# Shahriar1638/Hybrid-Language-Music-Clustering-VAE

Hardware: AMD Instinct MI355X
Metric: clips/sec mel+VAE train step, 128-mel x 128-frame, bs=256, 1/2/4/8 MI355X (higher is better)
Workload: dtype bf16; 1 GPU; Convolutional_VAE audio-only (BASELINE config[1]): PCM[256,65024] -> HIP mel-dB 128x128 -> z-score -> VAE fwd+bwd+Adam; per_gpu_batch=256, global_batch=256, mel=128x128, params=13304961, parallelism=dp1, world_size=1, launch=single process, pcm_batches=5 distinct batches in rotation (333 MB), execution=eager launches

## Files before the change

hybrid-language-music-clustering-vae_amd/_lib.py:

```python
from __future__ import annotations

import ctypes as C
import os

import torch

_HERE = os.path.dirname(os.path.abspath(__file__))
LIB_PATH = os.environ.get("HLMC_LIB") or os.path.join(_HERE, "libhlmc.so")

c_int, c_i64, c_f32, c_f64, c_vp, c_char_p = C.c_int, C.c_int64, C.c_float, C.c_double, C.c_void_p, C.c_char_p
P_vp = C.POINTER(c_vp)
P_i64 = C.POINTER(c_i64)

HLMC_F32, HLMC_BF16 = 0, 1
NET_HYBRID, NET_CVAE, NET_SIMPLE = 0, 1, 2

_SIGS = {
    "hlmc_version": (c_int, []),
    "hlmc_last_error": (c_char_p, []),
    "hlmc_device_status": (c_int, [c_int]),
    "hlmc_test_bn_fused": (c_int, [c_i64, c_int]),
    "hlmc_mel_plan_create": (c_int, [c_int, c_int, c_int, c_int, c_f64, c_f64, P_vp]),
    "hlmc_mel_plan_destroy": (c_int, [c_vp]),
    "hlmc_mel_filterbank": (c_int, [c_vp, c_vp]),
# ... 42 lines not shown
    "hlmc_probe_arm": (c_int, [c_int, c_int]),
    "hlmc_probe_read": (c_int, [C.POINTER(c_int), C.POINTER(c_f64), C.POINTER(c_f64), C.POINTER(c_f64),
                                C.POINTER(c_f32), c_int]),
    "hlmc_loss_workspace": (c_i64, [c_i64, c_i64, c_i64]),
    "hlmc_loss_sums": (c_int, [c_vp, c_vp, c_vp, c_i64, c_vp, c_vp, c_i64, c_vp, c_vp, c_i64, c_vp, c_vp]),
    "hlmc_loss_backward": (c_int, [c_vp, c_vp, c_vp, c_i64, c_vp, c_vp, c_vp, c_i64, c_vp, c_vp, c_vp, c_i64,
                                   c_vp, c_vp, c_vp]),
    "hlmc_loss_sums_backward": (c_int, [c_vp, c_vp, c_vp, c_i64, c_vp, c_vp, c_vp, c_i64, c_vp, c_vp, c_vp, c_i64,
                                        c_vp, c_vp, c_vp, c_vp, c_vp]),
    "hlmc_adam_scratch_bytes": (c_i64, [c_int]),
    "hlmc_adam_step": (c_int, [c_vp, c_int, P_vp, P_vp, P_vp, P_vp, P_i64, c_f32, c_f32, c_f32, c_f32, c_f32,
                               c_int, c_vp]),
    "hlmc_km_center": (c_int, [c_vp, c_vp, c_i64, c_int, c_vp, c_vp, c_vp]),
    "hlmc_km_sqdist_rows": (c_int, [c_vp, c_vp, c_i64, c_int, P_i64, c_int, c_vp]),
    "hlmc_km_assign": (c_int, [c_vp, c_vp, c_i64, c_int, c_vp, c_int, c_vp, c_vp, c_vp]),
    "hlmc_km_sums": (c_int, [c_vp, c_vp, c_i64, c_int, c_vp, c_int, c_vp, c_vp]),
    "hlmc_km_sums_workspace": (c_i64, [c_i64, c_int]),
    "hlmc_km_sums_part": (c_int, [c_vp, c_vp, c_i64, c_int, c_vp, c_int, c_vp, c_vp, c_vp, c_i64]),
    "hlmc_km_rowdist": (c_int, [c_vp, c_vp, c_i64, c_int, c_vp, c_vp, c_vp]),
    "hlmc_km_inertia": (c_int, [c_vp, c_vp, c_i64, c_int, c_vp, c_vp, c_vp, c_vp]),
    "hlmc_op_bn_bwd_workspace": (c_i64, [c_int]),
    "hlmc_op_bn_bwd": (c_int, [c_vp, c_int, c_vp, c_vp, c_i64, c_int, c_vp, c_vp, c_vp, c_vp, c_vp, c_vp, c_vp, c_vp, c_vp,
                               c_i64]),
    "hlmc_km_assign_batch": (c_int, [c_vp, c_vp, c_i64, c_int, c_vp, c_int, c_int, C.c_uint64, c_vp, c_vp, c_vp]),
    "hlmc_km_sums_batch": (c_int, [c_vp, c_vp, c_i64, c_int, c_vp, c_int, c_int, C.c_uint64, c_vp, c_vp, c_vp, c_i64]),
    "hlmc_km_update_batch": (c_int, [c_vp, c_int, c_int, c_int, C.c_uint64, c_vp, c_vp, c_vp, c_vp, c_vp]),
    "hlmc_km_pp_search": (c_int, [c_vp, c_i64, c_int, c_int, c_vp, c_int, C.POINTER(C.c_int32), C.POINTER(c_f64), c_vp,
                                  c_vp]),
    "hlmc_km_pp_dist": (c_int, [c_vp, c_vp, c_i64, c_int, c_int, c_int, c_vp, c_vp, c_int, C.POINTER(C.c_int32), c_vp]),
    "hlmc_km_inertia_batch": (c_int, [c_vp, c_vp, c_i64, c_int, c_vp, c_int, c_vp, c_int, c_vp, c_vp]),
    "hlmc_silhouette_workspace": (c_i64, [c_i64, c_int]),
    "hlmc_silhouette": (c_int, [c_vp, c_vp, c_i64, c_int, c_vp, c_int, c_vp, c_vp, c_vp, c_i64]),
    "hlmc_cluster_scores_workspace": (c_i64, [c_int, c_int]),
    "hlmc_cluster_scores": (c_int, [c_vp, c_vp, c_i64, c_int, c_vp, c_int, c_vp, c_vp, c_i64]),
    "hlmc_dbscan_workspace": (c_i64, [c_i64, c_int]),
    "hlmc_dbscan_neighbors": (c_int, [c_vp, c_vp, c_i64, c_int, C.POINTER(c_f64), c_int, c_vp, c_vp, c_vp, c_i64]),
    "hlmc_dbscan_labels": (c_int, [c_vp, c_i64, c_int, c_int, c_int, c_vp, c_vp, c_i64, c_vp, c_vp, c_vp]),
    "hlmc_ward_workspace": (c_i64, [c_i64]),
    "hlmc_ward_pdist": (c_int, [c_vp, c_vp, c_i64, c_int, c_vp]),
    "hlmc_ward_chain": (c_int, [c_vp, c_i64, c_vp, c_vp, c_vp, c_vp, c_vp, c_vp, c_i64]),
    "hlmc_op_conv_s2": (c_int, [c_vp, c_int, c_vp, c_int, c_int, c_int, c_int, c_vp, c_vp, c_int, c_vp, c_vp, c_i64]),
    "hlmc_op_subpixel": (c_int, [c_vp, c_int, c_vp, c_int, c_int, c_int, c_int, c_vp, c_vp, c_int, c_vp, c_vp, c_i64]),
    "hlmc_op_wgrad_s2": (c_int, [c_vp, c_int, c_vp, c_int, c_int, c_int, c_int, c_vp, c_int, c_vp, c_vp, c_i64]),
    "hlmc_op_linear": (c_int, [c_vp, c_int, c_vp, c_int, c_int, c_int, c_vp, c_int, c_vp, c_int, c_vp, c_int, c_int,
                               c_int, c_int, c_vp, c_i64, c_vp]),
    "hlmc_op_linear_wgrad": (c_int, [c_vp, c_int, c_vp, c_int, c_vp, c_int, c_int, c_int, c_int, c_vp, c_vp, c_vp,
# ... 78 lines not shown
```

hybrid-language-music-clustering-vae_amd/csrc/capi.cpp:

```cpp
#include <algorithm>
#include <cmath>
#include <cstring>
#include <memory>
#include <vector>

#include "engine.hpp"
#include "features.hpp"

namespace hlmc {

static thread_local std::string g_err;
void set_error(const std::string& msg) { g_err = msg; }
const char* get_error() { return g_err.c_str(); }
static int device_status_ok() {
    const unsigned st = ops::dev_status_take(false);
    if (st == 0) return HLMC_OK;
    set_error("device status " + std::to_string(st) +
              (st & kDevBnCountTimeout ? ": a one-launch BatchNorm backward's grid-wide arrival count timed out (grid not "
                                         "co-resident); that launch's dgamma / dbeta / dy are NaN" : "") +
              " -- clear with hlmc_device_status(1)");
    return HLMC_EDEVICE;
}

namespace probe {
// ... 493 lines not shown
    if (C <= 0) return 0;
    return (int64_t)(((ops::bn_acc_bytes(C) + 255) & ~(size_t)255) + ((ops::bias_acc_bytes(C) + 255) & ~(size_t)255) +
                     2 * (size_t)C * sizeof(float));
}
int hlmc_op_bn_bwd(void* stream, int dtype, const void* da, const void* y, int64_t R, int C, const float* mean,
                   const float* invstd, const float* gamma, const float* beta, void* dy, float* dgamma, float* dbeta,
                   float* dbias, void* ws, int64_t ws_bytes) {
    HLMC_CHECK_ARG(da && y && mean && invstd && gamma && beta && dy && dgamma && dbeta && ws && R > 1 && C > 0,
                   "hlmc_op_bn_bwd: arguments");
    HLMC_CHECK_ARG(ws_bytes >= hlmc_op_bn_bwd_workspace(C), "hlmc_op_bn_bwd: workspace too small");
    HLMC_TRY(device_status_ok());
    hipStream_t s = S(stream);
    unsigned char* w = static_cast<unsigned char*>(ws);
    const size_t o1 = (ops::bn_acc_bytes(C) + 255) & ~(size_t)255, o2 = o1 + ((ops::bias_acc_bytes(C) + 255) & ~(size_t)255);
    HLMC_HIP(hipMemsetAsync(ws, 0, o2, s));
    XAcc mom{reinterpret_cast<unsigned long long*>(w), xacc_shards(C), 2 * C};
    XAcc bacc{reinterpret_cast<unsigned long long*>(w + o1), xacc_shards(C), C};
    float* sums = reinterpret_cast<float*>(w + o2);
    return DT_DISPATCH(dtype,
        ops::bn_act_bwd<float>(s, (const float*)da, C, (const float*)y, R, C, mean, invstd, gamma, beta, 0, nullptr,
                               1.f, (float*)dy, dgamma, dbeta, mom, nullptr, dbias ? bacc : XAcc{}, dbias, sums),
        ops::bn_act_bwd<bf16>(s, (const bf16*)da, C, (const bf16*)y, R, C, mean, invstd, gamma, beta, 0, nullptr, 1.f,
                              (bf16*)dy, dgamma, dbeta, mom, nullptr, dbias ? bacc : XAcc{}, dbias, sums));
}
static size_t halo_acc_off(int Ci) { return (XAcc::bytes(xacc_shards(Ci), 2 * Ci) + 255) & ~(size_t)255; }
int64_t hlmc_op_halo_workspace(int Ci, int Co) {
    return (int64_t)(halo_acc_off(Ci) + XAcc::bytes(xacc_shards(Co), 2 * Co));
}
int hlmc_op_halo_fwd(void* stream, int kind, const void* x, int B, int Hi, int Wi, int Ci, const void* wp,
                     const float* bias, int Co, void* y, double* out_sums, const float* gamma, const float* beta,
                     float* running_mean, float* running_var, int64_t* num_batches_tracked, float momentum, float eps,
                     float* mean_out, float* invstd_out, void* a_out, void* ws, int64_t ws_bytes) {
    HLMC_CHECK_ARG(kind == 0 || kind == 1, "hlmc_op_halo_fwd: kind 0 (conv_s2) or 1 (subpixel)");
    HLMC_CHECK_ARG(out_sums && ws && ws_bytes >= hlmc_op_halo_workspace(Ci, Co), "hlmc_op_halo_fwd: workspace / out_sums");
    const bool xin = gamma != nullptr;
    HLMC_CHECK_ARG(kind == 0 ? ops::conv_s2_takes_input_bn<bf16>(B, Hi, Wi, Ci, Co)
                             : ops::subpixel_takes_input_bn<bf16>(B, Hi, Wi, Ci, Co),
                   "hlmc_op_halo_fwd: not an LDS halo-tile shape");
    if (xin) HLMC_CHECK_ARG(beta && mean_out && invstd_out && a_out, "hlmc_op_halo_fwd: input BatchNorm arguments");
    hipStream_t s = S(stream);
    unsigned char* w = static_cast<unsigned char*>(ws);
    XAcc ain{reinterpret_cast<unsigned long long*>(w), xacc_shards(Ci), 2 * Ci};
    XAcc aout{reinterpret_cast<unsigned long long*>(w + halo_acc_off(Ci)), xacc_shards(Co), 2 * Co};
    HLMC_HIP(hipMemsetAsync(ws, 0, (size_t)hlmc_op_halo_workspace(Ci, Co), s));
    const int64_t R = (int64_t)B * Hi * Wi;
    ops::BnInput bi{};
// ... 20 lines not shown
```

hybrid-language-music-clustering-vae_amd/csrc/engine.cpp:

```cpp
#include "engine.hpp"

#include <algorithm>
#include <climits>
#include <cstdlib>
#include <functional>

namespace hlmc {
namespace {

constexpr float kBnEps = 1e-5f;
constexpr float kBnMomentum = 0.1f;
constexpr int ENC_CH[7] = {1, 32, 64, 128, 256, 512, 512};
constexpr int DEC_CH[7] = {512, 512, 256, 128, 64, 32, 1};

inline int pad8(int64_t n) { return (int)((n + 7) & ~int64_t(7)); }

struct WgradQueue {
    using Fn = std::function<int(hipStream_t, Ws)>;
    bool on = true;
    Ws ws_main{nullptr, 0};
    Ws ws_own{nullptr, 0};

    WgradQueue() = default;
    WgradQueue(const WgradQueue&) = delete;
// ... 442 lines not shown
        int C = 0;
        float* gb = nullptr;
    };
    int bn_bwd(hipStream_t s, const T* da, int lda, const T* y, int64_t R, int C, const BnBufs& bb, int g, int beta,
               int act, const uint8_t* mask, float mscale, T* dy, int bias, const ops::BnBwdFuse* fused = nullptr,
               PendingBias* to_wgrad = nullptr) {
        const bool hand_off = bias >= 0 && wq.on && to_wgrad;
        const XAcc bacc = bias >= 0 ? acc_bias(bb) : XAcc{};
        if (to_wgrad) *to_wgrad = hand_off ? PendingBias{bacc, C, G[bias]} : PendingBias{};
        return ops::bn_act_bwd<T>(s, da, lda, y, R, C, AF(bb.mean), AF(bb.inv), P[g], P[beta], act, mask, mscale, dy,
                                  G[g], G[beta], acc_mom(bb), fused, bacc,
                                  (bias >= 0 && !hand_off) ? G[bias] : nullptr, AF(bb.sums));
    }
    ops::BnBwdFuse fuse4{};

    struct Enc {
        int w[6], b[6], g[6], beta[6], bn[6];
        int H = 0, W = 0;
        int rows(int l) const { return H >> l; }
        int cols(int l) const { return W >> l; }
        size_t y[6], a[6], dy[6];
        const float* audio = nullptr;
        BnBufs bb[6];
    };
    Enc enc;
    void enc_register(const std::string& prefix) {
        for (int l = 0; l < 6; ++l) {
            const int ci = ENC_CH[l], co = ENC_CH[l + 1];
            enc.w[l] = add_param(prefix + "." + std::to_string(3 * l) + ".weight", {co, ci, 3, 3});
            enc.b[l] = add_param(prefix + "." + std::to_string(3 * l) + ".bias", {co});
            enc.g[l] = add_param(prefix + "." + std::to_string(3 * l + 1) + ".weight", {co});
            enc.beta[l] = add_param(prefix + "." + std::to_string(3 * l + 1) + ".bias", {co});
            enc.bn[l] = add_bn();
            if (l > 0) register_pack(enc.w[l], 9);
        }
    }
    void enc_plan(Arena& A, int64_t B) {
        for (int l = 0; l < 6; ++l) {
            const int ci = ENC_CH[l], co = ENC_CH[l + 1];
            const int h = enc.rows(l), w = enc.cols(l), ho = enc.rows(l + 1), wo = enc.cols(l + 1);
            if (l > 0) {
                need(ops::conv_s2_ws<T>((int)B, h, w, ci, co));
                need(ops::subpixel_ws<T>((int)B, ho, wo, co, ci));
                need(ops::wgrad_s2_ws<T>((int)B, ho, wo, co, ci));
            } else {
                need(ops::wgrad_c1_ws((int)B, ho, wo, co));
            }
            const size_t n = (size_t)B * ho * wo * co;
            enc.y[l] = A.take(n * sizeof(T));
            enc.a[l] = l < 5 ? A.take(n * sizeof(T)) : 0;
            enc.dy[l] = A.take(n * sizeof(T));
            enc.bb[l] = bn_plan(A, co);
        }
    }
    size_t enc_max_elems(int64_t B) const { return (size_t)B * enc.rows(1) * enc.cols(1) * 32; }
    ops::BnInput bn_input(const BnBufs& bb, int bn, int g, int beta, int64_t R, size_t a_off) {
        return ops::BnInput{{acc_fwd(bb), R, AF(bb.mean), AF(bb.inv), RM[bn], RV[bn], NBT[bn], kBnMomentum, kBnEps},
                            P[g], P[beta], ws + a_off};
    }
    int enc_fwd(hipStream_t s, bool train, const float* audio_in, int B, T* flat, int ldflat) {
        HLMC_CHECK_ARG(audio_in, "audio input required");
        const float* audio = audio_in;
        enc.audio = audio_in;
        bool fused_prev = false;
        ops::BnInput xin{};
        for (int l = 0; l < 6; ++l) {
            const int ci = ENC_CH[l], co = ENC_CH[l + 1];
            const int h = enc.rows(l), w = enc.cols(l), ho = enc.rows(l + 1), wo = enc.cols(l + 1);
            T* y = AT(enc.y[l]);
            ops::ColStats st{train ? acc_fwd(enc.bb[l]) : XAcc{}, false};
            if (l == 0)
                HLMC_TRY(ops::conv_c1_s2<T>(s, audio, B, h, w, P[enc.w[0]], P[enc.b[0]], co, y, &st));
            else
                HLMC_TRY(ops::conv_s2<T>(s, fused_prev ? AT(enc.y[l - 1]) : AT(enc.a[l - 1]), B, h, w, ci, P0(enc.w[l]),
                                         P[enc.b[l]], co, y, scratch, &st, fused_prev ? &xin : nullptr));
            const int64_t R = (int64_t)B * ho * wo;
            fused_prev = train && l + 1 < 6 && ops::conv_s2_takes_input_bn<T>(B, ho, wo, co, ENC_CH[l + 2]);
            if (fused_prev) {
                if (!st.done) HLMC_TRY(ops::bn_moments<T>(s, y, R, co, acc_fwd(enc.bb[l])));
                xin = bn_input(enc.bb[l], enc.bn[l], enc.g[l], enc.beta[l], R, enc.a[l]);
            } else if (l == 5) {
                const ops::FlatOut fo{ldflat, nullptr};
                HLMC_TRY(bn_fwd(s, train, y, R, co, enc.bn[l], enc.bb[l], enc.g[l], enc.beta[l], 0, nullptr, 1.f, flat, 0,
                                &st, &fo, ho * wo));
            } else
                HLMC_TRY(bn_fwd(s, train, y, R, co, enc.bn[l], enc.bb[l], enc.g[l], enc.beta[l], 0, nullptr, 1.f,
                                AT(enc.a[l]), co, &st));
        }
        return HLMC_OK;
    }
    int enc_bwd(hipStream_t s, int B, T* gA, int bucket_hi = -1) {
        const float* audio = enc.audio;
        HLMC_CHECK_ARG(audio, "backward: no forward input recorded");
        for (int l = 5; l >= 0; --l) {
            const int ci = ENC_CH[l], co = ENC_CH[l + 1];
            const int ho = enc.rows(l + 1), wo = enc.cols(l + 1);
            const int64_t R = (int64_t)B * ho * wo;
            T* dy = AT(enc.dy[l]);
            PendingBias pb;
            HLMC_TRY(bn_bwd(s, gA, co, AT(enc.y[l]), R, co, enc.bb[l], enc.g[l], enc.beta[l], 0, nullptr, 1.f, dy, enc.b[l],
                            nullptr, &pb));
            float* gw = G[enc.w[l]];
            if (l == 0) {
                if (pb.gb) HLMC_TRY(ops::colsum_finalize(s, pb.acc, pb.C, pb.gb));
                HLMC_TRY(ops::wgrad_c1<T>(s, dy, B, ho, wo, co, audio, gw, scratch));
            } else {
                const T* xin = AT(enc.a[l - 1]);
                HLMC_TRY(wq.queue(s, [=](hipStream_t q, Ws sc) {
                    return ops::wgrad_s2<T>(q, dy, B, ho, wo, co, xin, ci, gw, sc, pb.acc, pb.gb);
                }, side_batch()));
                if (l == 1) HLMC_TRY(wq.flush(s));
                HLMC_TRY(ops::subpixel<T>(s, dy, B, ho, wo, co, P1(enc.w[l]), nullptr, ci, gA, scratch));
            }
            if (l == 3 && bucket_hi >= 0) HLMC_TRY(mark(s, bucket_hi));
            if (l == 2) HLMC_TRY(prelate(s));
        }
        return HLMC_OK;
    }

    struct Dec {
// ... 704 lines not shown
```

hybrid-language-music-clustering-vae_amd/csrc/kernels.hip:

```cpp
#include "ops.hpp"

#include <algorithm>
#include <cmath>
#include <cstdlib>
#include <cstring>
#include <map>
#include <mutex>
#include <tuple>
#include <type_traits>
#include <vector>
#include <atomic>

namespace hlmc {
namespace {

constexpr int kThreads = 256;
constexpr int kC1FusedBlocks = 1024;
constexpr int kC1BwdBlocks = 768;

inline int grid_for(int64_t n, int per_block = kThreads, int cap = 8192) {
    return (int)std::max<int64_t>(1, std::min<int64_t>(cap, (n + per_block - 1) / per_block));
}

constexpr int kBnBlockTarget = 1024;
// ... 974 lines not shown
            for (int j = 0; j < 9; ++j) red[wave][lane][i * 9 + j] = acc[i][j];
    }
    __syncthreads();
    for (int o = tid; o < M * 9; o += 256) {
        const int co = o / 9, tap = o - co * 9, g = co >> 3, i = co & 7;
        const float v = (red[0][g][i * 9 + tap] + red[1][g][i * 9 + tap]) + (red[2][g][i * 9 + tap] + red[3][g][i * 9 + tap]);
        part[(int64_t)blockIdx.x * (M * 9) + o] = v;
    }
}

__global__ __launch_bounds__(256) void sum_partials_f32_kernel(const float* __restrict__ part, int nblk, int n,
                                                               float* out) {
    __shared__ double sh[256];
    const int i = blockIdx.x;
    double s = 0.0;
    for (int k = threadIdx.x; k < nblk; k += blockDim.x) s += part[(int64_t)k * n + i];
    sh[threadIdx.x] = s;
    __syncthreads();
    for (int w = blockDim.x / 2; w > 0; w >>= 1) {
        if ((int)threadIdx.x < w) sh[threadIdx.x] += sh[threadIdx.x + w];
        __syncthreads();
    }
    if (threadIdx.x == 0) out[i] = (float)sh[0];
}

template <typename TI, typename TO>
__global__ void cast_kernel(const TI* __restrict__ x, TO* __restrict__ y, int64_t n) {
    for (int64_t i = (int64_t)blockIdx.x * blockDim.x + threadIdx.x; i < n; i += (int64_t)gridDim.x * blockDim.x)
        y[i] = from_f32<TO>(to_f32<TI>(x[i]));
}
template <typename TI, typename TO>
__global__ void cast2d_kernel(const TI* __restrict__ x, int ldx, TO* __restrict__ y, int ldy, int rows, int cols) {
    int64_t n = (int64_t)rows * cols;
    for (int64_t i = (int64_t)blockIdx.x * blockDim.x + threadIdx.x; i < n; i += (int64_t)gridDim.x * blockDim.x) {
        int r = (int)(i / cols), c = (int)(i % cols);
        y[(int64_t)r * ldy + c] = from_f32<TO>(to_f32<TI>(x[(int64_t)r * ldx + c]));
    }
}
struct LatentOut {
    float* mu = nullptr;
    float* lv = nullptr;
    float* eps = nullptr;
};
template <typename T>
__global__ void reparam_fwd_kernel(const float* __restrict__ mu, const float* __restrict__ lv,
                                   const float* __restrict__ eps, int n_rows, int L, T* __restrict__ z, int ldz,
// ... 740 lines not shown
        const int64_t rows = (int64_t)B * Hl;
        HLMC_CHECK_ARG(rows < (int64_t)1 << 31, "wgrad_c1: too many rows");
        const int nb = wgrad_c1_row_blocks(rows);
        HLMC_CHECK_ARG(ws.bytes >= (size_t)nb * M * 9 * sizeof(float), "wgrad_c1 workspace");
        wgrad_c1_rows_kernel<T><<<nb, kThreads, 0, s>>>(L, (int)rows, Hl, Xh, ws.p);
        HLMC_LAUNCHED();
        sum_partials_f32_kernel<<<M * 9, 256, 0, s>>>(ws.p, nb, M * 9, dW);
        HLMC_LAUNCHED();
        return HLMC_OK;
    }
    int64_t K = (int64_t)B * Hl * Wl;
    int nblk = wgrad_c1_blocks(K);
    HLMC_CHECK_ARG(ws.bytes >= wgrad_c1_ws(B, Hl, Wl, M), "wgrad_c1 workspace");
    int rpb = (int)((K + nblk - 1) / nblk);
    HLMC_CHECK_ARG(K < (int64_t)1 << 31, "wgrad_c1: too many rows");
    wgrad_c1_kernel<T, 32><<<nblk, kThreads, 0, s>>>(L, B, Hl, Wl, Xh, rpb, ws.p, FastDiv((uint32_t)Wl),
                                                     FastDiv((uint32_t)Hl));
    HLMC_LAUNCHED();
    sum_partials_f32_kernel<<<M * 9, 256, 0, s>>>(ws.p, nblk, M * 9, dW);
    HLMC_LAUNCHED();
    return HLMC_OK;
}

template <typename T>
int cast_from_f32(hipStream_t s, const float* x, T* y, int64_t n) {
    cast_kernel<float, T><<<grid_for(n), kThreads, 0, s>>>(x, y, n);
    HLMC_LAUNCHED();
    return HLMC_OK;
}
template <typename T>
int cast_to_f32(hipStream_t s, const T* x, float* y, int64_t n) {
    cast_kernel<T, float><<<grid_for(n), kThreads, 0, s>>>(x, y, n);
    HLMC_LAUNCHED();
    return HLMC_OK;
}
template <typename T>
int copy2d(hipStream_t s, const T* x, int ldx, T* y, int ldy, int rows, int cols) {
    cast2d_kernel<T, T><<<grid_for((int64_t)rows * cols), kThreads, 0, s>>>(x, ldx, y, ldy, rows, cols);
    HLMC_LAUNCHED();
    return HLMC_OK;
}
template <typename T>
int cast2d_from_f32(hipStream_t s, const float* x, int ldx, T* y, int ldy, int rows, int cols) {
    cast2d_kernel<float, T><<<grid_for((int64_t)rows * cols), kThreads, 0, s>>>(x, ldx, y, ldy, rows, cols);
    HLMC_LAUNCHED();
    return HLMC_OK;
// ... 229 lines not shown
int pack(hipStream_t s, const AdamJob* jobs_dev, int njobs, int total_tiles) {
    if (njobs == 0 || total_tiles == 0) return HLMC_OK;
    pack_kernel<T><<<total_tiles, 256, 0, s>>>(jobs_dev, njobs);
    HLMC_LAUNCHED();
    return HLMC_OK;
}

#define INST(T)                                                                                                      \
    template int bn_stats<T>(hipStream_t, const T*, int64_t, int, float*, float*, float*, float*, int64_t*, float,     \
                             float, XAcc);                                                                            \
    template int bn_moments<T>(hipStream_t, const T*, int64_t, int, XAcc);                                             \
    template int bn_act<T>(hipStream_t, const T*, int64_t, int, const float*, const float*, const float*, const float*, \
                           int, const uint8_t*, float, T*, int, const FlatOut*, int);                                 \
    template int bn_act_train<T>(hipStream_t, const T*, int64_t, int, XAcc, bool, float*, float*, float*,            \
                                 float*, int64_t*, float, float, const float*, const float*, int, const uint8_t*, float, \
                                 T*, int, const FlatOut*, int);                                                      \
    template int bn_act_bwd<T>(hipStream_t, const T*, int, const T*, int64_t, int, const float*, const float*,          \
                               const float*, const float*, int, const uint8_t*, float, T*, float*, float*, XAcc,      \
                               const BnBwdFuse*, XAcc, float*, float*);                                              \
    template int conv_c1_s2<T>(hipStream_t, const float*, int, int, int, const float*, const float*, int, T*,        \
                               ColStats*, BnBwdFuse*);                                                               \
    template int convT_c1<T>(hipStream_t, const T*, int, int, int, int, const float*, const float*, float*);         \
    template int wgrad_c1<T>(hipStream_t, const T*, int, int, int, int, const float*, float*, Ws);                    \
    template int cast_from_f32<T>(hipStream_t, const float*, T*, int64_t);                                           \
    template int cast_to_f32<T>(hipStream_t, const T*, float*, int64_t);                                             \
    template int copy2d<T>(hipStream_t, const T*, int, T*, int, int, int);                                           \
    template int cast2d_from_f32<T>(hipStream_t, const float*, int, T*, int, int, int);                              \
    template int heads_reparam<T>(hipStream_t, const float*, int, int, int, const float*, const float*, float*,      \
                                  float*, float*, float*, const float*, uint64_t, uint64_t, float*, T*, int);        \
    template int reparam_bwd_reduce<T>(hipStream_t, const float*, int, int, int, const float*, const float*,         \
                                       const float*, const float*, T*, T*, int);                                     \
    template int colsum<T>(hipStream_t, const T*, int, int, int, float*, Ws);                                        \
    template int reparam_fwd<T>(hipStream_t, const float*, const float*, const float*, int, int, T*, int, float*,     \
                                float*, float*);                                                                     \
    template int reparam_rng<T>(hipStream_t, const float*, const float*, uint64_t, uint64_t, int, int, float*, T*, int, \
                                float*, float*);                                                                     \
    template int reparam_bwd<T>(hipStream_t, const T*, int, const float*, const float*, const float*, const float*,  \
                                int, int, T*, T*);                                                                  \
    template int pack<T>(hipStream_t, const AdamJob*, int, int);                                                     \
    template int adam_pack<T>(hipStream_t, const AdamJob*, int, int, AdamArgs, const float*, int);

INST(float)
INST(bf16)
#undef INST

}
// ... 2 lines not shown
```

hybrid-language-music-clustering-vae_amd/csrc/ops.hpp:

```cpp
#pragma once
#include "common.hpp"

namespace hlmc {

struct Ws {
    float* p;
    size_t bytes;
};

namespace ops {

struct ColStats {
    XAcc acc;
    bool done;
};
struct BnBwdFuse {
    const void* y;
    const float *mean, *invstd, *gamma, *beta;
    XAcc acc;
    bool done;
};
struct BnInput : BnTrainFwd {
    const float *gamma = nullptr, *beta = nullptr;
    void* a_out = nullptr;
// ... 35 lines not shown
size_t linear_ws(int M, int K, int N);
template <typename T>
int linear_partials(hipStream_t s, const T* x, int ldx, int M, int K, const T* w, int ldw, int N, Ws ws, int* S_out);
template <typename T>
size_t linear_partials_ws(int M, int K, int N);

template <typename T>
int linear_wgrad(hipStream_t s, const T* dy, int lddy, const T* x, int ldx, int Mb, int N, int K, float* dW, float* db,
                 Ws ws);
template <typename T>
size_t linear_wgrad_ws(int Mb, int N, int K);
template <typename T>
int linear_wgrad_pair(hipStream_t s, const T* dy, int lddy, const T* x, int ldx, int Mb, int N1, int K, float* dW1,
                      float* db1, float* dW2, float* db2, Ws ws);

template <typename T>
int conv_c1_s2(hipStream_t s, const float* x, int B, int Hi, int Wi, const float* w, const float* bias, int Co, T* y,
               ColStats* st = nullptr, BnBwdFuse* bf = nullptr);
template <typename T>
int convT_c1(hipStream_t s, const T* x, int B, int Hi, int Wi, int Ci, const float* w, const float* bias, float* y);
template <typename T>
int wgrad_c1(hipStream_t s, const T* L, int B, int Hl, int Wl, int M, const float* Xh, float* dW, Ws ws);
size_t wgrad_c1_ws(int B, int Hl, int Wl, int M);

size_t bn_acc_bytes(int C);
size_t bias_acc_bytes(int C);
template <typename T>
int bn_stats(hipStream_t s, const T* y, int64_t R, int C, float* mean, float* invstd, float* run_mean, float* run_var,
             int64_t* nbt, float momentum, float eps, XAcc acc);
template <typename T>
int bn_moments(hipStream_t s, const T* y, int64_t R, int C, XAcc acc);
int bn_eval_stats(hipStream_t s, const float* run_mean, const float* run_var, int C, float eps, float* mean, float* invstd);
template <typename T>
int bn_act_train(hipStream_t s, const T* y, int64_t R, int C, XAcc acc, bool have_stats, float* mean, float* invstd,
                 float* run_mean, float* run_var, int64_t* nbt, float momentum, float eps, const float* gamma,
                 const float* beta, int act, const uint8_t* mask, float mscale, T* a, int lda,
                 const FlatOut* fo = nullptr, int hw = 0);
template <typename T>
int bn_act(hipStream_t s, const T* y, int64_t R, int C, const float* mean, const float* invstd, const float* gamma,
           const float* beta, int act, const uint8_t* mask, float mscale, T* a, int lda, const FlatOut* fo = nullptr,
           int hw = 0);
template <typename T>
int bn_act_bwd(hipStream_t s, const T* da, int lda, const T* y, int64_t R, int C, const float* mean, const float* invstd,
               const float* gamma, const float* beta, int act, const uint8_t* mask, float mscale, T* dy, float* dgamma,
               float* dbeta, XAcc mom, const BnBwdFuse* fused, XAcc bias_acc, float* dbias, float* sums);
int colsum_finalize(hipStream_t s, XAcc acc, int C, float* out);
// ... 72 lines not shown
```

include/hlmc.h:

```cpp
#ifndef HLMC_H_
#define HLMC_H_

#include <stdint.h>

#ifdef __cplusplus
extern "C" {
#endif

enum hlmc_status {
    HLMC_OK = 0,
    HLMC_EINVAL = -1,
    HLMC_EHIP = -2,
    HLMC_EUNSUP = -3,
    HLMC_EDEVICE = -4,
};

enum hlmc_dtype { HLMC_F32 = 0, HLMC_BF16 = 1 };

int hlmc_version(void);
const char* hlmc_last_error(void);
int hlmc_device_status(int clear);
int hlmc_test_bn_fused(int64_t max_elems, int spin_max);

typedef struct hlmc_mel_plan hlmc_mel_plan;
// ... 133 lines not shown


int hlmc_op_conv_s2(void* stream, int dtype, const void* x, int B, int Hi, int Wi, int Ci, const void* wp,
                    const float* bias, int Co, void* y, void* ws, int64_t ws_bytes);
int hlmc_op_subpixel(void* stream, int dtype, const void* x, int B, int Hi, int Wi, int Ci, const void* wp,
                     const float* bias, int Co, void* y, void* ws, int64_t ws_bytes);
int hlmc_op_wgrad_s2(void* stream, int dtype, const void* L, int B, int Hl, int Wl, int M, const void* Xh, int C,
                     float* dW, void* ws, int64_t ws_bytes);
int hlmc_op_linear(void* stream, int dtype, const void* x, int ldx, int M, int K, const void* w, int ldw,
                   const float* bias, int N, void* y, int ldy, int act, int accumulate, int out_f32, void* ws,
                   int64_t ws_bytes, const void* relu_ref);
int hlmc_op_linear_wgrad(void* stream, int dtype, const void* dy, int lddy, const void* x, int ldx, int Mb, int N,
                         int K, float* dW, float* db, void* ws, int64_t ws_bytes);
int hlmc_op_conv_c1_s2(void* stream, int dtype, const float* x, int B, int Hi, int Wi, const float* w,
                       const float* bias, int Co, void* y);
int hlmc_op_convT_c1(void* stream, int dtype, const void* x, int B, int Hi, int Wi, int Ci, const float* w,
                     const float* bias, float* y);
int hlmc_op_wgrad_c1(void* stream, int dtype, const void* L, int B, int Hl, int Wl, int M, const float* Xh,
                     float* dW, void* ws, int64_t ws_bytes);
int64_t hlmc_op_bn_bwd_workspace(int C);
int hlmc_op_bn_bwd(void* stream, int dtype, const void* da, const void* y, int64_t R, int C, const float* mean,
                   const float* invstd, const float* gamma, const float* beta, void* dy, float* dgamma, float* dbeta,
                   float* dbias, void* ws, int64_t ws_bytes);
int64_t hlmc_op_halo_workspace(int Ci, int Co);
int hlmc_op_halo_fwd(void* stream, int kind, const void* x, int B, int Hi, int Wi, int Ci, const void* wp,
                     const float* bias, int Co, void* y, double* out_sums, const float* gamma, const float* beta,
                     float* running_mean, float* running_var, int64_t* num_batches_tracked, float momentum, float eps,
                     float* mean_out, float* invstd_out, void* a_out, void* ws, int64_t ws_bytes);

#ifdef __cplusplus
}
#endif
#endif
```

Baseline: 144,200 clips/s.

## Fuse first-layer BN backward with conv weight-gradient via tap Gram algebra

For the first encoder layer (single input channel, 64-wide maps, 32 outputs), one row kernel now runs the BatchNorm backward and accumulates the per-tap products dz·x alongside the BN moment sums. The dy tensor is never written, and the separate weight-gradient pass over it is gone. The BN correction terms are applied afterwards in a single-block finalize kernel. That kernel uses a 9x9 Gram matrix of the input taps, computed on a side queue, to reconstruct the needed cross terms algebraically. This saves one full-size write and read of the layer-0 gradient at the cost of extra accumulators and a double-precision finalize with different rounding.

```diff
diff --git a/hybrid-language-music-clustering-vae_amd/_lib.py b/hybrid-language-music-clustering-vae_amd/_lib.py
--- a/hybrid-language-music-clustering-vae_amd/_lib.py
+++ b/hybrid-language-music-clustering-vae_amd/_lib.py
@@ -88,6 +88,9 @@
     "hlmc_op_bn_bwd_workspace": (c_i64, [c_int]),
     "hlmc_op_bn_bwd": (c_int, [c_vp, c_int, c_vp, c_vp, c_i64, c_int, c_vp, c_vp, c_vp, c_vp, c_vp, c_vp, c_vp, c_vp, c_vp,
                                c_i64]),
+    "hlmc_op_bn_bwd_wgrad_c1_workspace": (c_i64, []),
+    "hlmc_op_bn_bwd_wgrad_c1": (c_int, [c_vp, c_int, c_vp, c_vp, c_int, c_int, c_int, c_vp, c_vp, c_vp, c_vp, c_vp, c_vp,
+                                        c_vp, c_vp, c_vp, c_vp, c_vp, c_vp, c_i64]),
     "hlmc_km_assign_batch": (c_int, [c_vp, c_vp, c_i64, c_int, c_vp, c_int, c_int, C.c_uint64, c_vp, c_vp, c_vp]),
     "hlmc_km_sums_batch": (c_int, [c_vp, c_vp, c_i64, c_int, c_vp, c_int, c_int, C.c_uint64, c_vp, c_vp, c_vp, c_i64]),
     "hlmc_km_update_batch": (c_int, [c_vp, c_int, c_int, c_int, C.c_uint64, c_vp, c_vp, c_vp, c_vp, c_vp]),
diff --git a/hybrid-language-music-clustering-vae_amd/csrc/capi.cpp b/hybrid-language-music-clustering-vae_amd/csrc/capi.cpp
--- a/hybrid-language-music-clustering-vae_amd/csrc/capi.cpp
+++ b/hybrid-language-music-clustering-vae_amd/csrc/capi.cpp
@@ -539,6 +539,34 @@
                                1.f, (float*)dy, dgamma, dbeta, mom, nullptr, dbias ? bacc : XAcc{}, dbias, sums),
         ops::bn_act_bwd<bf16>(s, (const bf16*)da, C, (const bf16*)y, R, C, mean, invstd, gamma, beta, 0, nullptr, 1.f,
                               (bf16*)dy, dgamma, dbeta, mom, nullptr, dbias ? bacc : XAcc{}, dbias, sums));
+}
+static size_t al256(size_t b) { return (b + 255) & ~(size_t)255; }
+int64_t hlmc_op_bn_bwd_wgrad_c1_workspace(void) {
+    return (int64_t)(al256(ops::bn_acc_bytes(32)) + al256(ops::c1_bwd_acc_bytes()) + al256(ops::c1_gram_acc_bytes()));
+}
+int hlmc_op_bn_bwd_wgrad_c1(void* stream, int dtype, const void* da, const void* y, int B, int Hl, int Wl,
+                            const float* mean, const float* invstd, const float* gamma, const float* beta,
+                            const float* audio, const float* w, const float* bias, float* dW, float* dbias,
+                            float* dgamma, float* dbeta, void* ws, int64_t ws_bytes) {
+    HLMC_CHECK_ARG(da && y && mean && invstd && gamma && beta && audio && w && dW && dgamma && dbeta && ws,
+                   "hlmc_op_bn_bwd_wgrad_c1: arguments");
+    HLMC_CHECK_ARG(ws_bytes >= hlmc_op_bn_bwd_wgrad_c1_workspace(), "hlmc_op_bn_bwd_wgrad_c1: workspace too small");
+    HLMC_CHECK_ARG(DT_DISPATCH(dtype, ops::bn_bwd_wgrad_c1_ok<float>(B, Hl, Wl, 32, 0),
+                               ops::bn_bwd_wgrad_c1_ok<bf16>(B, Hl, Wl, 32, 0)),
+                   "hlmc_op_bn_bwd_wgrad_c1: only 64-wide maps");
+    hipStream_t s = S(stream);
+    unsigned char* p = static_cast<unsigned char*>(ws);
+    const size_t o1 = al256(ops::bn_acc_bytes(32)), o2 = o1 + al256(ops::c1_bwd_acc_bytes());
+    HLMC_HIP(hipMemsetAsync(ws, 0, (size_t)hlmc_op_bn_bwd_wgrad_c1_workspace(), s));
+    const XAcc mom{reinterpret_cast<unsigned long long*>(p), xacc_shards(32), 64};
+    const XAcc a = ops::c1_bwd_acc(p + o1), gram = ops::c1_gram_acc(p + o2);
+    HLMC_TRY(ops::c1_tap_gram(s, audio, B, Hl, Wl, gram));
+    HLMC_TRY(DT_DISPATCH(dtype,
+        ops::bn_bwd_wgrad_c1<float>(s, (const float*)da, (const float*)y, B, Hl, Wl, 32, mean, invstd, gamma, beta, 0,
+                                    audio, mom, a),
+        ops::bn_bwd_wgrad_c1<bf16>(s, (const bf16*)da, (const bf16*)y, B, Hl, Wl, 32, mean, invstd, gamma, beta, 0,
+                                   audio, mom, a)));
+    return ops::bn_bwd_c1_finalize(s, B, Hl, Wl, mom, a, gram, mean, invstd, gamma, w, bias, dW, dbias, dgamma, dbeta);
 }
 static size_t halo_acc_off(int Ci) { return (XAcc::bytes(xacc_shards(Ci), 2 * Ci) + 255) & ~(size_t)255; }
 int64_t hlmc_op_halo_workspace(int Ci, int Co) {
diff --git a/hybrid-language-music-clustering-vae_amd/csrc/engine.cpp b/hybrid-language-music-clustering-vae_amd/csrc/engine.cpp
--- a/hybrid-language-music-clustering-vae_amd/csrc/engine.cpp
+++ b/hybrid-language-music-clustering-vae_amd/csrc/engine.cpp
@@ -488,6 +488,8 @@
         size_t y[6], a[6], dy[6];
         const float* audio = nullptr;
         BnBufs bb[6];
+        bool one_pass0 = false;
+        size_t xa0 = 0, xgram0 = 0;
     };
     Enc enc;
     void enc_register(const std::string& prefix) {
@@ -515,8 +517,15 @@
             const size_t n = (size_t)B * ho * wo * co;
             enc.y[l] = A.take(n * sizeof(T));
             enc.a[l] = l < 5 ? A.take(n * sizeof(T)) : 0;
-            enc.dy[l] = A.take(n * sizeof(T));
+            if (l == 0) enc.one_pass0 = ops::bn_bwd_wgrad_c1_ok<T>((int)B, ho, wo, co, 0);
+            enc.dy[l] = l == 0 && enc.one_pass0 ? 0 : A.take(n * sizeof(T));
             enc.bb[l] = bn_plan(A, co);
+            if (l == 0 && enc.one_pass0) {
+                enc.xa0 = xb_total;
+                xb_total += al256(ops::c1_bwd_acc_bytes());
+                enc.xgram0 = xb_total;
+                xb_total += al256(ops::c1_gram_acc_bytes());
+            }
         }
     }
     size_t enc_max_elems(int64_t B) const { return (size_t)B * enc.rows(1) * enc.cols(1) * 32; }
@@ -558,10 +567,28 @@
     int enc_bwd(hipStream_t s, int B, T* gA, int bucket_hi = -1) {
         const float* audio = enc.audio;
         HLMC_CHECK_ARG(audio, "backward: no forward input recorded");
+        const XAcc gram0 = ops::c1_gram_acc(ws + xb_base + enc.xgram0);
+        if (enc.one_pass0) {
+            const int h1 = enc.rows(1), w1 = enc.cols(1);
+            HLMC_TRY(wq.run(s, [=](hipStream_t q, Ws) { return ops::c1_tap_gram(q, audio, B, h1, w1, gram0); }));
+        }
         for (int l = 5; l >= 0; --l) {
             const int ci = ENC_CH[l], co = ENC_CH[l + 1];
             const int ho = enc.rows(l + 1), wo = enc.cols(l + 1);
             const int64_t R = (int64_t)B * ho * wo;
+            if (l == 0 && enc.one_pass0) {
+                const BnBufs& bb = enc.bb[0];
+                const XAcc mom = acc_mom(bb), a0 = ops::c1_bwd_acc(ws + xb_base + enc.xa0);
+                const float *mean = AF(bb.mean), *inv = AF(bb.inv), *gam = P[enc.g[0]];
+                HLMC_TRY(ops::bn_bwd_wgrad_c1<T>(s, gA, AT(enc.y[0]), B, ho, wo, co, mean, inv, gam, P[enc.beta[0]], 0, audio,
+                                                 mom, a0));
+                const float *w0 = P[enc.w[0]], *b0 = P[enc.b[0]];
+                float *gw0 = G[enc.w[0]], *gb0 = G[enc.b[0]], *gg0 = G[enc.g[0]], *gbeta0 = G[enc.beta[0]];
+                HLMC_TRY(wq.run(s, [=](hipStream_t q, Ws) {
+                    return ops::bn_bwd_c1_finalize(q, B, ho, wo, mom, a0, gram0, mean, inv, gam, w0, b0, gw0, gb0, gg0, gbeta0);
+                }));
+                break;
+            }
             T* dy = AT(enc.dy[l]);
             PendingBias pb;
             HLMC_TRY(bn_bwd(s, gA, co, AT(enc.y[l]), R, co, enc.bb[l], enc.g[l], enc.beta[l], 0, nullptr, 1.f, dy, enc.b[l],
diff --git a/hybrid-language-music-clustering-vae_amd/csrc/kernels.hip b/hybrid-language-music-clustering-vae_amd/csrc/kernels.hip
--- a/hybrid-language-music-clustering-vae_amd/csrc/kernels.hip
+++ b/hybrid-language-music-clustering-vae_amd/csrc/kernels.hip
@@ -1020,6 +1020,222 @@
         __syncthreads();
     }
     if (threadIdx.x == 0) out[i] = (float)sh[0];
+}
+
+constexpr int kC1Taps = 9, kC1Co = 32;
+constexpr int kC1ACols = kC1Co * kC1Taps + kC1Co;
+constexpr int kC1GramCols = kC1Taps + kC1Taps * (kC1Taps + 1) / 2;
+constexpr int kC1Shards = 16;
+__host__ __device__ constexpr int c1_gram_col(int i, int j) {
+    const int a = i < j ? i : j, b = i < j ? j : i;
+    return kC1Taps + a * kC1Taps - a * (a - 1) / 2 + (b - a);
+}
+
+__device__ __forceinline__ void c1_load_taps(const float* __restrict__ Xh, int row, int Hl, int c, float (&xv)[3][3]) {
+    constexpr int WH = 128;
+    const int b = row / Hl, r = row - b * Hl;
+#pragma unroll
+    for (int kh = 0; kh < 3; ++kh) {
+        const int ih = 2 * r - 1 + kh;
+        const float* xr = Xh + ((int64_t)b * 2 * Hl + (ih < 0 ? 0 : ih)) * WH + 2 * c;
+        const float2 lo = *reinterpret_cast<const float2*>(xr - (c > 0 ? 2 : 0));
+        const float2 hi = *reinterpret_cast<const float2*>(xr);
+        const bool okr = ih >= 0;
+        xv[kh][0] = (okr && c > 0) ? lo.y : 0.f;
+        xv[kh][1] = okr ? hi.x : 0.f;
+        xv[kh][2] = okr ? hi.y : 0.f;
+    }
+}
+
+template <typename T>
+__global__ __launch_bounds__(256, 2) void bn_bwd_wgrad_c1_rows_kernel(
+    const T* __restrict__ da, const T* __restrict__ y, int rows, int Hl, const float* __restrict__ Xh,
+    const float* __restrict__ mean, const float* __restrict__ invstd, const float* __restrict__ gamma,
+    const float* __restrict__ beta, XAcc mom, XAcc aacc) {
+    constexpr int WL = 64, M = kC1Co, U = 4, NS = 8 * 9 + 3 * 8;
+    __shared__ double red[4][4][NS];
+    const int tid = threadIdx.x, c = tid >> 2, cg = tid & 3, lane = tid & 63, wave = tid >> 6;
+    float mu[8], is[8], ga[8], be[8];
+    BnChan::load(mean, 8 * cg, mu);
+    BnChan::load(invstd, 8 * cg, is);
+    BnChan::load(gamma, 8 * cg, ga);
+    BnChan::load(beta, 8 * cg, be);
+    float acc[8][9], fa[8], fb[8], fc[8];
+#pragma unroll
+    for (int i = 0; i < 8; ++i) {
+        fa[i] = fb[i] = fc[i] = 0.f;
+#pragma unroll
+        for (int j = 0; j < 9; ++j) acc[i][j] = 0.f;
+    }
+    const int stride = gridDim.x;
+    for (int r0 = blockIdx.x; r0 < rows; r0 += U * stride) {
+        float gv[U][8], yv[U][8], xv[U][3][3];
+#pragma unroll
+        for (int u = 0; u < U; ++u) {
+            const int row = r0 + u * stride < rows ? r0 + u * stride : 0;
+            const int64_t o = ((int64_t)row * WL + c) * M + 8 * cg;
+            if constexpr (sizeof(T) == 2) {
+                cvt16_f32<T>(load16_raw(da + o), gv[u]);
+                cvt16_f32<T>(load16_raw(y + o), yv[u]);
+            } else {
+                cvt16_f32<T>(load16_raw(da + o), gv[u]);
+                cvt16_f32<T>(load16_raw(da + o + 4), gv[u] + 4);
+                cvt16_f32<T>(load16_raw(y + o), yv[u]);
+                cvt16_f32<T>(load16_raw(y + o + 4), yv[u] + 4);
+            }
+            c1_load_taps(Xh, row, Hl, c, xv[u]);
+        }
+#pragma unroll
+        for (int u = 0; u < U; ++u) {
+            const bool valid = r0 + u * stride < rows;
+#pragma unroll
+            for (int i = 0; i < 8; ++i) {
+                float xh = (yv[u][i] - mu[i]) * is[i];
+                float z = xh * ga[i] + be[i];
+                float dz = gv[u][i] * act_grad_t<0>(z, 0);
+                dz = valid ? dz : 0.f;
+                fa[i] += dz;
+                fb[i] = fmaf(dz, xh, fb[i]);
+                fc[i] += valid ? xh : 0.f;
+#pragma unroll
+                for (int kh = 0; kh < 3; ++kh)
+#pragma unroll
+                    for (int kw = 0; kw < 3; ++kw) acc[i][kh * 3 + kw] = fmaf(dz, xv[u][kh][kw], acc[i][kh * 3 + kw]);
+            }
+        }
+    }
+#pragma unroll
+    for (int i = 0; i < 8; ++i)
+#pragma unroll
+        for (int j = 0; j < 9; ++j) {
+            double v = acc[i][j];
+#pragma unroll
+            for (int o = 4; o < 64; o <<= 1) v += __shfl_xor(v, o, 64);
+            if (lane < 4) red[wave][lane][i * 9 + j] = v;
+        }
+#pragma unroll
+    for (int i = 0; i < 8; ++i) {
+        double a = fa[i], b = fb[i], d = fc[i];
+#pragma unroll
+        for (int o = 4; o < 64; o <<= 1) {
+            a += __shfl_xor(a, o, 64);
+            b += __shfl_xor(b, o, 64);
+            d += __shfl_xor(d, o, 64);
+        }
+        if (lane < 4) {
+            red[wave][lane][72 + i] = a;
+            red[wave][lane][80 + i] = b;
+            red[wave][lane][88 + i] = d;
+        }
+    }
+    __syncthreads();
+    for (int o = tid; o < kC1ACols + 2 * M; o += 256) {
+        int co, slot;
+        if (o < M * 9) {
+            co = o / 9;
+            slot = (co & 7) * 9 + (o - co * 9);
+        } else {
+            const int k = (o - M * 9) / M;
+            co = (o - M * 9) - k * M;
+            slot = (k == 0 ? 88 : k == 1 ? 72 : 80) + (co & 7);
+        }
+        const int g = co >> 3;
+        const double v = (red[0][g][slot] + red[1][g][slot]) + (red[2][g][slot] + red[3][g][slot]);
+        if (o < kC1ACols)
+            xacc_add(aacc, o, v);
+        else
+            xacc_add(mom, o - kC1ACols, v);
+    }
+}
+
+__global__ __launch_bounds__(256) void c1_tap_gram_kernel(const float* __restrict__ Xh, int rows, int Hl, XAcc gacc) {
+    constexpr int NG = kC1GramCols;
+    __shared__ double red[4][NG];
+    const int tid = threadIdx.x, c = tid & 63, wave = tid >> 6;
+    float sx[9], pr[NG - 9];
+#pragma unroll
+    for (int i = 0; i < 9; ++i) sx[i] = 0.f;
+#pragma unroll
+    for (int i = 0; i < NG - 9; ++i) pr[i] = 0.f;
+    for (int row = blockIdx.x * 4 + wave; row < rows; row += gridDim.x * 4) {
+        float xv[3][3];
+        c1_load_taps(Xh, row, Hl, c, xv);
+        const float t[9] = {xv[0][0], xv[0][1], xv[0][2], xv[1][0], xv[1][1], xv[1][2], xv[2][0], xv[2][1], xv[2][2]};
+#pragma unroll
+        for (int i = 0; i < 9; ++i) {
+            sx[i] += t[i];
+#pragma unroll
+            for (int j = 0; j < 9; ++j)
+                if (j >= i) pr[c1_gram_col(i, j) - 9] = fmaf(t[i], t[j], pr[c1_gram_col(i, j) - 9]);
+        }
+    }
+#pragma unroll
+    for (int i = 0; i < 9; ++i) {
+        const double v = wave_sum((double)sx[i]);
+        if (c == 0) red[wave][i] = v;
+#pragma unroll
+        for (int j = 0; j < 9; ++j)
+            if (j >= i) {
+                const double p = wave_sum((double)pr[c1_gram_col(i, j) - 9]);
+                if (c == 0) red[wave][c1_gram_col(i, j)] = p;
+            }
+    }
+    __syncthreads();
+    if (tid < NG) xacc_add(gacc, tid, (red[0][tid] + red[1][tid]) + (red[2][tid] + red[3][tid]));
+}
+
+__device__ __forceinline__ double c1_xacc_column(const XAcc& acc, int c) {
+    unsigned long long w0[kC1Shards], w1[kC1Shards], w2[kC1Shards];
+#pragma unroll
+    for (int sh = 0; sh < kC1Shards; ++sh) {
+        const unsigned long long* q = acc.p + (size_t)sh * 3 * acc.ncols + c;
+        w0[sh] = q[0];
+        w1[sh] = q[acc.ncols];
+        w2[sh] = q[2 * acc.ncols];
+    }
+    long long a = 0, b = 0, d = 0;
+    unsigned long long bad = 0;
+#pragma unroll
+    for (int sh = 0; sh < kC1Shards; ++sh) {
+        a += (long long)w0[sh];
+        b += (long long)w1[sh];
+        bad |= w2[sh] & kXAccBad;
+        d += (long long)(w2[sh] & ~kXAccBad);
+    }
+    return bad ? __builtin_nan("") : xacc_value(a, b, d);
+}
+constexpr int kC1FinThreads = kC1ACols + 2 * kC1Co + 64;
+__global__ __launch_bounds__(kC1FinThreads) void bn_bwd_c1_finalize_kernel(XAcc mom, XAcc aacc, XAcc gacc, int64_t R,
+                                                                     const float* __restrict__ mean,
+                                                                     const float* __restrict__ invstd,
+                                                                     const float* __restrict__ gamma,
+                                                                     const float* __restrict__ w,
+                                                                     const float* __restrict__ bias, float* dW,
+                                                                     float* dbias, float* dgamma, float* dbeta) {
+    constexpr int M = kC1Co;
+    __shared__ double sa[kC1ACols], sm[2 * M], sg[kC1GramCols];
+    const int t = threadIdx.x;
+    if (t < kC1ACols)
+        sa[t] = c1_xacc_column(aacc, t);
+    else if (t < kC1ACols + 2 * M)
+        sm[t - kC1ACols] = c1_xacc_column(mom, t - kC1ACols);
+    else if (t < kC1ACols + 2 * M + kC1GramCols)
+        sg[t - kC1ACols - 2 * M] = c1_xacc_column(gacc, t - kC1ACols - 2 * M);
+    __syncthreads();
+    if (t >= kC1ACols) return;
+    const int c = t < M * 9 ? t / 9 : t - M * 9;
+    const double k = (double)gamma[c] * (double)invstd[c], mg = sm[c] / (double)R, mgx = sm[M + c] / (double)R;
+    if (t < M * 9) {
+        const int tap = t - c * 9;
+        double syx = (bias ? (double)bias[c] : 0.0) * sg[tap];
+        for (int j = 0; j < 9; ++j) syx += (double)w[c * 9 + j] * sg[c1_gram_col(j, tap)];
+        const double sxh = (double)invstd[c] * (syx - (double)mean[c] * sg[tap]);
+        dW[t] = (float)(k * (sa[t] - mg * sg[tap] - mgx * sxh));
+    } else {
+        dbeta[c] = (float)sm[c];
+        dgamma[c] = (float)sm[M + c];
+        if (dbias) dbias[c] = (float)(k * (sm[c] - (double)R * mg - mgx * sa[t]));
+    }
 }
 
 template <typename TI, typename TO>
@@ -1806,6 +2022,53 @@
     return HLMC_OK;
 }
 
+size_t c1_bwd_acc_bytes() { return XAcc::bytes(kC1Shards, kC1ACols); }
+size_t c1_gram_acc_bytes() { return XAcc::bytes(kC1Shards, kC1GramCols); }
+XAcc c1_bwd_acc(void* p) { return XAcc{static_cast<unsigned long long*>(p), kC1Shards, kC1ACols}; }
+XAcc c1_gram_acc(void* p) { return XAcc{static_cast<unsigned long long*>(p), kC1Shards, kC1GramCols}; }
+template <typename T>
+bool bn_bwd_wgrad_c1_ok(int B, int Hl, int Wl, int Co, int act) {
+    return B > 0 && Hl > 0 && Wl == 64 && Co == kC1Co && act == 0 && (int64_t)B * Hl < (int64_t)1 << 31;
+}
+int c1_tap_gram(hipStream_t s, const float* audio, int B, int Hl, int Wl, XAcc gram) {
+    HLMC_CHECK_ARG(audio && ((uintptr_t)audio & 15) == 0 && Wl == 64 && (int64_t)B * Hl < (int64_t)1 << 31,
+                   "c1_tap_gram: 64-wide maps, 16-byte-aligned audio");
+    HLMC_TRY(check_acc(gram, kC1GramCols));
+    const int rows = B * Hl;
+    c1_tap_gram_kernel<<<std::min(1024, cdiv(rows, 4)), kThreads, 0, s>>>(audio, rows, Hl, gram);
+    HLMC_LAUNCHED();
+    return HLMC_OK;
+}
+template <typename T>
+int bn_bwd_wgrad_c1(hipStream_t s, const T* da, const T* y, int B, int Hl, int Wl, int Co, const float* mean,
+                    const float* invstd, const float* gamma, const float* beta, int act, const float* audio, XAcc mom,
+                    XAcc aacc) {
+    HLMC_CHECK_ARG(bn_bwd_wgrad_c1_ok<T>(B, Hl, Wl, Co, act), "bn_bwd_wgrad_c1: shape");
+    HLMC_CHECK_ARG((((uintptr_t)da | (uintptr_t)y | (uintptr_t)audio) & 15) == 0, "bn_bwd_wgrad_c1: alignment");
+    HLMC_TRY(check_acc(mom, 2 * Co));
+    HLMC_TRY(check_acc(aacc, kC1ACols));
+    const int rows = B * Hl;
+    HLMC_BN_PROBED(s, 2.0 * sizeof(T) * rows * 64 * Co + 16.0 * rows * 64,
+                   (bn_bwd_wgrad_c1_rows_kernel<T><<<wgrad_c1_row_blocks(rows), kThreads, 0, s>>>(
+                       da, y, rows, Hl, audio, mean, invstd, gamma, beta, mom, aacc)));
+    HLMC_LAUNCHED();
+    return HLMC_OK;
+}
+int bn_bwd_c1_finalize(hipStream_t s, int B, int Hl, int Wl, XAcc mom, XAcc aacc, XAcc gram, const float* mean,
+                       const float* invstd, const float* gamma, const float* w, const float* bias, float* dW,
+                       float* dbias, float* dgamma, float* dbeta) {
+    HLMC_CHECK_ARG(mean && invstd && gamma && w && dW && dgamma && dbeta, "bn_bwd_c1_finalize: arguments");
+    HLMC_TRY(check_acc(mom, 2 * kC1Co));
+    HLMC_TRY(check_acc(aacc, kC1ACols));
+    HLMC_TRY(check_acc(gram, kC1GramCols));
+    HLMC_CHECK_ARG(mom.shards == kC1Shards && aacc.shards == kC1Shards && gram.shards == kC1Shards,
+                   "bn_bwd_c1_finalize: accumulator shards");
+    bn_bwd_c1_finalize_kernel<<<1, kC1FinThreads, 0, s>>>(mom, aacc, gram, (int64_t)B * Hl * Wl, mean, invstd, gamma, w, bias,
+                                                     dW, dbias, dgamma, dbeta);
+    HLMC_LAUNCHED();
+    return HLMC_OK;
+}
+
 template <typename T>
 int cast_from_f32(hipStream_t s, const float* x, T* y, int64_t n) {
     cast_kernel<float, T><<<grid_for(n), kThreads, 0, s>>>(x, y, n);
@@ -2081,6 +2344,9 @@
                                ColStats*, BnBwdFuse*);                                                               \
     template int convT_c1<T>(hipStream_t, const T*, int, int, int, int, const float*, const float*, float*);         \
     template int wgrad_c1<T>(hipStream_t, const T*, int, int, int, int, const float*, float*, Ws);                    \
+    template bool bn_bwd_wgrad_c1_ok<T>(int, int, int, int, int);                                                    \
+    template int bn_bwd_wgrad_c1<T>(hipStream_t, const T*, const T*, int, int, int, int, const float*, const float*,  \
+                                    const float*, const float*, int, const float*, XAcc, XAcc);                      \
     template int cast_from_f32<T>(hipStream_t, const float*, T*, int64_t);                                           \
     template int cast_to_f32<T>(hipStream_t, const T*, float*, int64_t);                                             \
     template int copy2d<T>(hipStream_t, const T*, int, T*, int, int, int);                                           \
diff --git a/hybrid-language-music-clustering-vae_amd/csrc/ops.hpp b/hybrid-language-music-clustering-vae_amd/csrc/ops.hpp
--- a/hybrid-language-music-clustering-vae_amd/csrc/ops.hpp
+++ b/hybrid-language-music-clustering-vae_amd/csrc/ops.hpp
@@ -81,6 +81,20 @@
 template <typename T>
 int wgrad_c1(hipStream_t s, const T* L, int B, int Hl, int Wl, int M, const float* Xh, float* dW, Ws ws);
 size_t wgrad_c1_ws(int B, int Hl, int Wl, int M);
+size_t c1_bwd_acc_bytes();
+size_t c1_gram_acc_bytes();
+XAcc c1_bwd_acc(void* p);
+XAcc c1_gram_acc(void* p);
+template <typename T>
+bool bn_bwd_wgrad_c1_ok(int B, int Hl, int Wl, int Co, int act);
+int c1_tap_gram(hipStream_t s, const float* audio, int B, int Hl, int Wl, XAcc gram);
+template <typename T>
+int bn_bwd_wgrad_c1(hipStream_t s, const T* da, const T* y, int B, int Hl, int Wl, int Co, const float* mean,
+                    const float* invstd, const float* gamma, const float* beta, int act, const float* audio, XAcc mom,
+                    XAcc a);
+int bn_bwd_c1_finalize(hipStream_t s, int B, int Hl, int Wl, XAcc mom, XAcc a, XAcc gram, const float* mean,
+                       const float* invstd, const float* gamma, const float* w, const float* bias, float* dW,
+                       float* dbias, float* dgamma, float* dbeta);
 
 size_t bn_acc_bytes(int C);
 size_t bias_acc_bytes(int C);
diff --git a/include/hlmc.h b/include/hlmc.h
--- a/include/hlmc.h
+++ b/include/hlmc.h
@@ -179,6 +179,11 @@
 int hlmc_op_bn_bwd(void* stream, int dtype, const void* da, const void* y, int64_t R, int C, const float* mean,
                    const float* invstd, const float* gamma, const float* beta, void* dy, float* dgamma, float* dbeta,
                    float* dbias, void* ws, int64_t ws_bytes);
+int64_t hlmc_op_bn_bwd_wgrad_c1_workspace(void);
+int hlmc_op_bn_bwd_wgrad_c1(void* stream, int dtype, const void* da, const void* y, int B, int Hl, int Wl,
+                            const float* mean, const float* invstd, const float* gamma, const float* beta,
+                            const float* audio, const float* w, const float* bias, float* dW, float* dbias,
+                            float* dgamma, float* dbeta, void* ws, int64_t ws_bytes);
 int64_t hlmc_op_halo_workspace(int Ci, int Co);
 int hlmc_op_halo_fwd(void* stream, int kind, const void* x, int B, int Hi, int Wi, int Ci, const void* wp,
                      const float* bias, int Co, void* y, double* out_sums, const float* gamma, const float* beta,
```

Measured after the change: 144,400 clips/s (median of 5 runs). No clear change (+0.1%).
